# ISU-PAAL/DeepDFA

Hardware: NVIDIA H100
Metric: CFG graphs/sec (train step) (higher is better)
Workload: dtype f32 (GRU GEMMs: bf16x3 split operands, f32 accumulate)

## Files before the change

### deepdfa_b200/csrc/gru_tc_bwd.cu

```cuda
#include <cuda_fp16.h>

#include <atomic>

#include "tc_common.cuh"

namespace ddfa {
namespace tc2b {
using namespace tcc;

constexpr int kThreads = 320, kEpiWarps = 8;

constexpr int kGbWarps = 8;
struct GbRow {
  float4 d, hv, rr, zz, nn, gh;
  float deg;
  int tb, te;
};
__device__ __forceinline__ float4 bf16x4_to_f4(const uint2 &p) {
  return make_float4(__uint_as_float(p.x << 16), __uint_as_float(p.x & 0xffff0000u), __uint_as_float(p.y << 16), __uint_as_float(p.y & 0xffff0000u));
}
__device__ __forceinline__ void gb_load(GbRow &x, const float *__restrict__ dh_out, const float *__restrict__ h,
                                        const uint8_t *__restrict__ h_img_src, const float *__restrict__ gates,
                                        const uint4 *__restrict__ gates_packed, const int32_t *__restrict__ indptr,
                                        const int32_t *__restrict__ indptr_t, size_t plane, int64_t node, int col, bool ok,
                                        uint64_t pol_saved, uint64_t pol_dh) {
  x.tb = x.te = 0;
  if (ok) {
    if (indptr_t) { x.tb = __ldcg(indptr_t + node); x.te = __ldcg(indptr_t + node + 1); }
    const size_t off = (size_t)node * kD + col;
    x.d = ldg_cg_f4_hint(dh_out + off, pol_dh);
    uint2 hh = make_uint2(0u, 0u), hl = hh;
    uint4 g0 = make_uint4(0u, 0u, 0u, 0u), g1 = g0;
    if (h) x.hv = ldg_cg_f4_hint(h + off, pol_saved);
    else {
      hh = __ldcg(reinterpret_cast<const uint2 *>(h_img_src + image_offset(node, col, 0)));
      hl = __ldcg(reinterpret_cast<const uint2 *>(h_img_src + image_offset(node, col, 1)));
    }
    if (gates) {
      x.rr = ldg_cg_f4_hint(gates + off, pol_saved);
      x.zz = ldg_cg_f4_hint(gates + plane + off, pol_saved);
      x.nn = ldg_cg_f4_hint(gates + 2 * plane + off, pol_saved);
      x.gh = ldg_cg_f4_hint(gates + 3 * plane + off, pol_saved);
    } else {
      g0 = __ldcg(gates_packed + (off >> 1));
      g1 = __ldcg(gates_packed + (off >> 1) + 1);
    }
    x.deg = (float)(__ldcg(indptr + node + 1) - __ldcg(indptr + node));
    if (!h) {
      const float4 a = bf16x4_to_f4(hh), b = bf16x4_to_f4(hl);
      x.hv = make_float4(a.x + b.x, a.y + b.y, a.z + b.z, a.w + b.w);
    }
    if (!gates) {
      unpack_gates(make_uint2(g0.x, g0.y), x.rr.x, x.zz.x, x.nn.x, x.gh.x);
      unpack_gates(make_uint2(g0.z, g0.w), x.rr.y, x.zz.y, x.nn.y, x.gh.y);
      unpack_gates(make_uint2(g1.x, g1.y), x.rr.z, x.zz.z, x.nn.z, x.gh.z);
      unpack_gates(make_uint2(g1.z, g1.w), x.rr.w, x.zz.w, x.nn.w, x.gh.w);
    }
  }
}

__global__ void __launch_bounds__(32 * kGbWarps, 2) gate_bwd_image_kernel(const float *__restrict__ dh_out, const float *__restrict__ h,
                                                                          const uint8_t *__restrict__ h_img_src,
                                                                          const float *__restrict__ gates, const uint4 *__restrict__ gates_packed,
                                                                          const int32_t *__restrict__ indptr,
                                                                          const float *__restrict__ ds_in, const int32_t *__restrict__ indptr_t,
                                                                          const int32_t *__restrict__ indices_t,
                                                                          int32_t N, uint8_t *__restrict__ q_img, size_t img_stride,
                                                                          uint8_t *__restrict__ h_img, float *__restrict__ dhz,
                                                                          float *__restrict__ db_fold,
                                                                          float *__restrict__ db_ih, float *__restrict__ db_hh, float *__restrict__ bias_slots,
                                                                          int hints) {
  __shared__ float red[kGbWarps][7 * kD];
  const int lane = threadIdx.x & 31, warp = threadIdx.x >> 5;
  const int col = lane * 4;
  pdl_launch_dependents();
  pdl_wait();
  const uint64_t pol_saved = l2_policy((hints & 2) ? 1 : 0), pol_tmp = l2_policy((hints & 4) ? 2 : 0), pol_dh = l2_policy((hints & 8) ? 1 : 0);
  const size_t plane = (size_t)N * kD;
  float4 sum[7];
#pragma unroll
  for (int i = 0; i < 7; ++i) sum[i] = make_float4(0.f, 0.f, 0.f, 0.f);
  const int64_t Npad = ((int64_t)N + kTileM - 1) / kTileM * kTileM;
  const int64_t stride = (int64_t)gridDim.x * kGbWarps;

  auto finish = [&](const GbRow &x, int64_t node, bool ok) {
    float4 qr = make_float4(0.f, 0.f, 0.f, 0.f), qz = qr, qn = qr, qnr = qr, hv = qr;
    if (ok) {
      hv = x.hv;
      st_f4_hint(dhz + (size_t)node * kD + col, make_float4(x.d.x * x.zz.x, x.d.y * x.zz.y, x.d.z * x.zz.z, x.d.w * x.zz.w), pol_tmp);
#define BWDQ(f)                                                      \
  {                                                                  \
    const float dz_ = x.d.f * (x.hv.f - x.nn.f);                     \
    const float dn_ = x.d.f * (1.f - x.zz.f);                        \
    qn.f = dn_ * (1.f - x.nn.f * x.nn.f);                            \
    qz.f = dz_ * x.zz.f * (1.f - x.zz.f);                            \
    qr.f = qn.f * x.gh.f * x.rr.f * (1.f - x.rr.f);                  \
    qnr.f = qn.f * x.rr.f;                                           \
  }
      BWDQ(x) BWDQ(y) BWDQ(z) BWDQ(w)
#undef BWDQ
      f4_add(sum[0], qr); f4_add(sum[1], qz); f4_add(sum[2], qn); f4_add(sum[3], qnr);
      f4_fma(sum[4], x.deg, qr); f4_fma(sum[5], x.deg, qz); f4_fma(sum[6], x.deg, qn);
    }
    const size_t o_hi = image_offset(node, col, 0), o_lo = image_offset(node, col, 1);
    uint2 ph, pl;
    split4(qr, ph, pl);  *reinterpret_cast<uint2 *>(q_img + 0 * img_stride + o_hi) = ph; *reinterpret_cast<uint2 *>(q_img + 0 * img_stride + o_lo) = pl;
    split4(qz, ph, pl);  *reinterpret_cast<uint2 *>(q_img + 1 * img_stride + o_hi) = ph; *reinterpret_cast<uint2 *>(q_img + 1 * img_stride + o_lo) = pl;
    split4(qn, ph, pl);  *reinterpret_cast<uint2 *>(q_img + 2 * img_stride + o_hi) = ph; *reinterpret_cast<uint2 *>(q_img + 2 * img_stride + o_lo) = pl;
    split4(qnr, ph, pl); *reinterpret_cast<uint2 *>(q_img + 3 * img_stride + o_hi) = ph; *reinterpret_cast<uint2 *>(q_img + 3 * img_stride + o_lo) = pl;
    if (h_img) {
      split4(hv, ph, pl); *reinterpret_cast<uint2 *>(h_img + o_hi) = ph; *reinterpret_cast<uint2 *>(h_img + o_lo) = pl;
    }
  };

  for (int64_t node = (int64_t)blockIdx.x * kGbWarps + warp; node < Npad; node += 2 * stride) {
    const int64_t node2 = node + stride;
    GbRow a, b;
    const bool ok_a = node < N, ok_b = node2 < N;
    gb_load(a, dh_out, h, h_img_src, gates, gates_packed, indptr, indptr_t, plane, node, col, ok_a, pol_saved, pol_dh);
    gb_load(b, dh_out, h, h_img_src, gates, gates_packed, indptr, indptr_t, plane, node2, col, ok_b, pol_saved, pol_dh);
    if (indptr_t) {
      int ia[4], ib[4];
#pragma unroll
      for (int k = 0; k < 4; ++k) {
        ia[k] = (a.tb + k < a.te) ? __ldcg(indices_t + a.tb + k) : -1;
        ib[k] = (b.tb + k < b.te) ? __ldcg(indices_t + b.tb + k) : -1;
      }
      float4 va[4], vb[4];
#pragma unroll
      for (int k = 0; k < 4; ++k) {
        va[k] = ia[k] >= 0 ? ldg_cg_f4(ds_in + (size_t)ia[k] * kD + col) : make_float4(0.f, 0.f, 0.f, 0.f);
        vb[k] = ib[k] >= 0 ? ldg_cg_f4(ds_in + (size_t)ib[k] * kD + col) : make_float4(0.f, 0.f, 0.f, 0.f);
      }
#pragma unroll
      for (int k = 0; k < 4; ++k) { f4_add(a.d, va[k]); f4_add(b.d, vb[k]); }
      for (int j = a.tb + 4; j < a.te; ++j) f4_add(a.d, ldg_cg_f4(ds_in + (size_t)__ldcg(indices_t + j) * kD + col));
      for (int j = b.tb + 4; j < b.te; ++j) f4_add(b.d, ldg_cg_f4(ds_in + (size_t)__ldcg(indices_t + j) * kD + col));
    }
    finish(a, node, ok_a);
    if (node2 < Npad) finish(b, node2, ok_b);
  }
#pragma unroll
  for (int i = 0; i < 7; ++i) *reinterpret_cast<float4 *>(&red[warp][i * kD + col]) = sum[i];
  __syncthreads();
  for (int i = threadIdx.x; i < 7 * kD; i += 32 * kGbWarps) {
    float v_ = 0.f;
#pragma unroll
    for (int w = 0; w < kGbWarps; ++w) v_ += red[w][i];
    if (bias_slots) { bias_slots[(size_t)blockIdx.x * 7 * kD + i] = v_; continue; }
    const int which = i >> 7, c_ = i & 127;
    if (which == 0) { atomicAdd(db_ih + c_, v_); atomicAdd(db_hh + c_, v_); }
    else if (which == 1) { atomicAdd(db_ih + kD + c_, v_); atomicAdd(db_hh + kD + c_, v_); }
    else if (which == 2) atomicAdd(db_ih + 2 * kD + c_, v_);
    else if (which == 3) atomicAdd(db_hh + 2 * kD + c_, v_);
    else atomicAdd(db_fold + (which - 4) * kD + c_, v_);
  }
}

constexpr int kD3Stages = 2;
constexpr int kD3StageBytes = kImageTileBytes;
constexpr int kD3WChunkBytes = 64 * 128;
constexpr int kD3WBytes = 12 * kD3WChunkBytes;
constexpr int kD3OffStage = kD3WBytes;
constexpr int kD3OffBar = kD3OffStage + kD3Stages * kD3StageBytes;
constexpr int kD3SmemAlloc = kD3OffBar + (2 * kD3Stages + 1) * 8 + 1024;
constexpr int kD3Threads = 32 * kEpiWarps + 32;
constexpr size_t kD3PackedBytes = (size_t)4 * kD3WBytes;
static_assert(kD3SmemAlloc <= 232448, "shared memory budget");

__global__ void dgrad3_pack_kernel(const float *__restrict__ w_fold, const float *__restrict__ w_hh, uint8_t *__restrict__ packed) {
  const int idx = blockIdx.x * blockDim.x + threadIdx.x;
  if (idx >= 4 * 3 * 64 * 16) return;
  const int u = idx % 16, n = (idx / 16) % 64, g = (idx / (16 * 64)) % 3, rh = idx / (16 * 64 * 3);
  const int role = rh >> 1, half = rh & 1, kb = u >> 3;
  const float *W = role == 0 ? w_fold : w_hh;
  float x[8];
#pragma unroll
  for (int i = 0; i < 8; ++i) x[i] = W[(size_t)(g * kD + u * 8 + i) * kD + half * 64 + n];
  uint4 ph, pl;
  split8(x, ph, pl);
  uint8_t *base = packed + (size_t)rh * kD3WBytes + sw128_offset(n, (u & 7) * 8);
  *reinterpret_cast<uint4 *>(base + ((g * 2 + 0) * 2 + kb) * kD3WChunkBytes) = ph;
  *reinterpret_cast<uint4 *>(base + ((g * 2 + 1) * 2 + kb) * kD3WChunkBytes) = pl;
}

__global__ void __launch_bounds__(kD3Threads, 1) dgrad3_kernel(const uint8_t *__restrict__ q_img, size_t img_stride,
                                                               const float *__restrict__ dhz, const uint8_t *__restrict__ packed3,
                                                               int32_t N, float *__restrict__ ds, float *__restrict__ dh, int hints) {
  extern __shared__ uint8_t smem_raw[];
  uint8_t *smem = reinterpret_cast<uint8_t *>((reinterpret_cast<uintptr_t>(smem_raw) + 1023) & ~(uintptr_t)1023);
  const uint32_t sbase = smem_u32(smem);
  const uint32_t bar0 = sbase + kD3OffBar;
  auto full = [&](int i) { return bar0 + 8u * i; };
  auto empty = [&](int i) { return bar0 + 8u * (kD3Stages + i); };
  const uint32_t w_full = bar0 + 8u * (2 * kD3Stages);
  const int tron = (g_trace_on == 1);

  const int warp = threadIdx.x >> 5, lane = threadIdx.x & 31;
  const int rh = blockIdx.x & 3, role = rh >> 1, half = rh & 1;
  const int group = blockIdx.x >> 2, num_groups = gridDim.x >> 2;
  const int num_tiles = (N + kTileM - 1) / kTileM;
  const int my_tiles = (num_tiles > group) ? (num_tiles - 1 - group) / num_groups + 1 : 0;

  if (threadIdx.x == 0) {
    for (int i = 0; i < kD3Stages; ++i) { mbar_init(full(i), 1); mbar_init(empty(i), kEpiWarps); }
    mbar_init(w_full, 1);
    mbar_fence_init();
  }
  __syncthreads();
  if (threadIdx.x == 0) trace_stamp(tron, 0, 0);
  pdl_launch_dependents();

  if (warp == kEpiWarps) {
    if (my_tiles > 0 && elect_one()) {
      mbar_arrive_expect_tx(w_full, kD3WBytes);
      bulk_g2s(sbase, packed3 + (size_t)rh * kD3WBytes, kD3WBytes, w_full);
      pdl_wait();
      const uint64_t pol_q = l2_policy((hints & 64) ? 1 : 0);
      int cc = 0;
      for (int k = 0; k < my_tiles; ++k) {
        const int tile = num_tiles - 1 - (group + k * num_groups);
        for (int g = 0; g < 3; ++g, ++cc) {
          const int m = g < 2 ? g : (role == 0 ? 2 : 3);
          const int stage = cc % kD3Stages, use = cc / kD3Stages;
          if (use > 0) mbar_wait_bounded(empty(stage), (use - 1) & 1);
          mbar_arrive_expect_tx(full(stage), kD3StageBytes);
          bulk_g2s_hint(sbase + kD3OffStage + stage * kD3StageBytes, q_img + (size_t)m * img_stride + (size_t)tile * kImageTileBytes,
                        kD3StageBytes, full(stage), pol_q);
          if (g != 1) trace_stamp(tron, k, g == 0 ? 1 : 2);
        }
      }
    }
    return;
  }

  pdl_wait();
  if (my_tiles == 0) return;
  const int wg = warp >> 2;
  const int row0 = wg * 64 + (warp & 3) * 16 + (lane >> 2);
  const int col0 = half * 64 + 2 * (lane & 3);
  float *out = role == 0 ? ds : dh;
  const uint64_t pol_tmp = l2_policy((hints & 4) ? 2 : 0);
  const uint64_t pol_dhz = l2_policy((hints & 8) ? 1 : 0);
  mbar_wait_bounded(w_full, 0);
  const bool tr = (warp == 0 && lane == 0);
  int cc = 0, pending = -1;
  for (int k = 0; k < my_tiles; ++k) {
    const int tile = num_tiles - 1 - (group + k * num_groups);
    float acc[32];
    if (tr) { trace_stamp(tron, k, 7); trace_stamp(tron, k, 3); }
    for (int g = 0; g < 3; ++g, ++cc) {
      const int stage = cc % kD3Stages, use = cc / kD3Stages;
      mbar_wait_bounded(full(stage), use & 1);
      if (tr && g != 1) trace_stamp(tron, k, g == 0 ? 4 : 5);
      wgmma_fence();
      const uint32_t a0 = sbase + kD3OffStage + stage * kD3StageBytes + wg * 8192;
      const uint32_t w0 = sbase + g * 4 * kD3WChunkBytes;
#pragma unroll
      for (int kb = 0; kb < 2; ++kb) {
#pragma unroll
        for (int k4 = 0; k4 < 4; ++k4) {
          const uint64_t a_hi = gmma_desc(a0 + kb * kChunkBytes + k4 * 32), a_lo = gmma_desc(a0 + (2 + kb) * kChunkBytes + k4 * 32);
          const uint64_t b_hi = gmma_desc(w0 + kb * kD3WChunkBytes + k4 * 32), b_lo = gmma_desc(w0 + (2 + kb) * kD3WChunkBytes + k4 * 32);
          wgmma_n64<0, 0>(acc, a_hi, b_hi, (g == 0 && kb == 0 && k4 == 0) ? 0u : 1u);
          wgmma_n64<0, 0>(acc, a_hi, b_lo, 1u);
          wgmma_n64<0, 0>(acc, a_lo, b_hi, 1u);
        }
      }
      wgmma_commit();
      wgmma_wait<1>();
      __syncwarp();
      if (pending >= 0 && lane == 0) mbar_arrive(empty(pending));
      pending = stage;
    }
    float2 dv[2][8];
#pragma unroll
    for (int hh = 0; hh < 2; ++hh) {
      const int64_t node = (int64_t)tile * kTileM + row0 + 8 * hh;
#pragma unroll
      for (int j = 0; j < 8; ++j) {
        dv[hh][j] = make_float2(0.f, 0.f);
        if (role == 1 && node < N) {
          const float *p = dhz + node * kD + col0 + 8 * j;
          dv[hh][j] = make_float2(ldg_cg_f32_hint(p, pol_dhz), ldg_cg_f32_hint(p + 1, pol_dhz));
        }
      }
    }
    wgmma_wait<0>();
    wgmma_fence_regs(acc);
    if (tr) { trace_stamp(tron, k, 6); trace_stamp(tron, k, 8); }
    __syncwarp();
    if (lane == 0) mbar_arrive(empty(pending));
    pending = -1;
    if (tr) trace_stamp(tron, k, 9);
#pragma unroll
    for (int hh = 0; hh < 2; ++hh) {
      const int64_t node = (int64_t)tile * kTileM + row0 + 8 * hh;
      if (node < N) {
#pragma unroll
        for (int j = 0; j < 8; ++j)
          st_f2_hint(out + node * kD + col0 + 8 * j, make_float2(acc[4 * j + 2 * hh] + dv[hh][j].x, acc[4 * j + 2 * hh + 1] + dv[hh][j].y), pol_tmp);
      }
    }
    if (tr) trace_stamp(tron, k, 10);
  }
}

constexpr int kGtRows = 32;
constexpr int kGtOffD = 0, kGtOffG = kGtRows * kD * 4, kGtOffH = kGtOffG + kGtRows * kD * 8;
static_assert(kGtOffH + kGtRows * kD * 4 == kD3StageBytes, "phase A's operands fill exactly one stage");
static_assert(4 * kGtRows == kTileM, "four CTAs per tile");
constexpr int kGtPre = 2;
constexpr int kGtRowsPerWarp = kGtRows / kEpiWarps;

__device__ __forceinline__ void fence_proxy_async_global() { asm volatile("fence.proxy.async.global;" ::: "memory"); }
__device__ __forceinline__ void cluster_arrive_release() { asm volatile("barrier.cluster.arrive.release;" ::: "memory"); }
__device__ __forceinline__ void cluster_wait_acquire() { asm volatile("barrier.cluster.wait.acquire;" ::: "memory"); }

template <bool HF32, bool CSRP>
__global__ void __launch_bounds__(kD3Threads, 1) bwd_step_fused_kernel(const float *__restrict__ dh_out, const float *__restrict__ h,
                                                                       const uint8_t *__restrict__ h_img_src, const uint2 *__restrict__ gates_packed,
                                                                       const int32_t *__restrict__ indptr, const float *__restrict__ ds_in,
                                                                       const int32_t *__restrict__ indptr_t, const int32_t *__restrict__ indices_t,
                                                                       int32_t N, uint8_t *__restrict__ q_img, size_t img_stride,
                                                                       const uint8_t *__restrict__ packed3, float *__restrict__ ds, float *__restrict__ dh,
                                                                       float *__restrict__ db_fold, float *__restrict__ db_ih, float *__restrict__ db_hh,
                                                                       float *__restrict__ bias_slots, int hints) {
  extern __shared__ uint8_t smem_raw[];
  uint8_t *smem = reinterpret_cast<uint8_t *>((reinterpret_cast<uintptr_t>(smem_raw) + 1023) & ~(uintptr_t)1023);
  const uint32_t sbase = smem_u32(smem);
  const uint32_t bar0 = sbase + kD3OffBar;
  auto full = [&](int i) { return bar0 + 8u * i; };
  auto empty = [&](int i) { return bar0 + 8u * (kD3Stages + i); };
  const uint32_t w_full = bar0 + 8u * (2 * kD3Stages);
  const int tron = (g_trace_on == 1);

  const int warp = threadIdx.x >> 5, lane = threadIdx.x & 31;
  const int rh = blockIdx.x & 3, role = rh >> 1, half = rh & 1;
  const int cluster = blockIdx.x >> 2, num_clusters = gridDim.x >> 2;
  const int num_tiles = (N + kTileM - 1) / kTileM;
  const int my_tiles = (num_tiles > cluster) ? (num_tiles - 1 - cluster) / num_clusters + 1 : 0;
  const int tile0 = num_tiles - 1 - cluster;
  auto tile_of = [&](int k) { return tile0 - k * num_clusters; };

  if (threadIdx.x == 0) {
    for (int i = 0; i < kD3Stages; ++i) { mbar_init(full(i), 1); mbar_init(empty(i), kEpiWarps); }
    mbar_init(w_full, 1);
    mbar_fence_init();
  }
  __syncthreads();
  if (threadIdx.x == 0) trace_stamp(tron, 0, 0);
  pdl_launch_dependents();

  if (warp == kEpiWarps) {
    const uint64_t pol_saved = l2_policy((hints & 2) ? 1 : 0), pol_dh = l2_policy((hints & 8) ? 1 : 0);
    const uint64_t pol_q = l2_policy((hints & 64) ? 1 : 0);
    if (my_tiles > 0 && elect_one()) {
      mbar_arrive_expect_tx(w_full, kD3WBytes);
      bulk_g2s(sbase, packed3 + (size_t)rh * kD3WBytes, kD3WBytes, w_full);
    }
    __syncwarp();
    pdl_wait();
    int cc = 0;
    for (int k = 0; k < my_tiles; ++k, cc += 4) {
      const int tile = tile_of(k);
      if (elect_one()) {
        const int stage = cc % kD3Stages, use = cc / kD3Stages;
        if (use > 0) mbar_wait_bounded(empty(stage), (use - 1) & 1);
        const int64_t r0 = (int64_t)tile * kTileM + kGtRows * rh;
        const int valid = (int)max((int64_t)0, min((int64_t)kGtRows, (int64_t)N - r0));
        const uint32_t dst = sbase + kD3OffStage + stage * kD3StageBytes;
        const uint32_t bytes = (uint32_t)valid * (kD * 4 + kD * 8) + (HF32 ? (uint32_t)valid * kD * 4 : (uint32_t)kGtRows * kD * 4);
        mbar_arrive_expect_tx(full(stage), bytes);
        if (valid > 0) {
          bulk_g2s_hint(dst + kGtOffD, dh_out + r0 * kD, (uint32_t)valid * kD * 4, full(stage), pol_dh);
          bulk_g2s_hint(dst + kGtOffG, gates_packed + r0 * kD, (uint32_t)valid * kD * 8, full(stage), pol_saved);
        }
        if (HF32) {
          if (valid > 0) bulk_g2s_hint(dst + kGtOffH, h + r0 * kD, (uint32_t)valid * kD * 4, full(stage), pol_saved);
        } else {
          const uint8_t *t0 = h_img_src + (size_t)tile * kImageTileBytes + (size_t)(kGtRows * rh) * 128;
#pragma unroll
          for (int ch = 0; ch < 4; ++ch) bulk_g2s_hint(dst + kGtOffH + ch * (kGtRows * 128), t0 + (size_t)ch * kChunkBytes, kGtRows * 128, full(stage), pol_saved);
        }
      }
      __syncwarp();
      cluster_arrive_release();
      cluster_wait_acquire();
      if (elect_one()) {
        fence_proxy_async_global();
        for (int g = 0; g < 3; ++g) {
          const int m = g < 2 ? g : (role == 0 ? 2 : 3);
          const int c = cc + 1 + g, stage = c % kD3Stages, use = c / kD3Stages;
          if (use > 0) mbar_wait_bounded(empty(stage), (use - 1) & 1);
          mbar_arrive_expect_tx(full(stage), kD3StageBytes);
          bulk_g2s_hint(sbase + kD3OffStage + stage * kD3StageBytes, q_img + (size_t)m * img_stride + (size_t)tile * kImageTileBytes,
                        kD3StageBytes, full(stage), pol_q);
          if (g != 1) trace_stamp(tron, k, g == 0 ? 1 : 2);
        }
      }
      __syncwarp();
    }
  } else {
    pdl_wait();
    const int col = lane * 4;
#define DDFA_POL_TMP l2_policy((hints & 4) ? 2 : 0)
#define DDFA_POL_DHZ l2_policy((hints & 8) ? 1 : 0)
    const int wg = warp >> 2;
    const int row0 = wg * 64 + (warp & 3) * 16 + (lane >> 2);
    const int col0 = half * 64 + 2 * (lane & 3);
    const bool tr = (warp == 0 && lane == 0);
    float4 sum[7];
#pragma unroll
    for (int i = 0; i < 7; ++i) sum[i] = make_float4(0.f, 0.f, 0.f, 0.f);
    static_assert(kGtPre == 2 && kGtRowsPerWarp == 4, "lane slots below assume four rows per warp and two prefetched neighbours per row");
    auto node_of = [&](int tile, int r) { return (int64_t)tile * kTileM + kGtRows * rh + warp + kEpiWarps * r; };
    auto load_scalars = [&](int kk) -> int {
      int v = 0;
      if (kk < my_tiles && lane < 16) {
        const int64_t nd = node_of(tile_of(kk), (lane >> 1) & 3);
        const int32_t *base = lane < 8 ? indptr : indptr_t;
        if (nd < N && base) v = __ldcg(base + nd + (lane & 1));
      }
      return v;
    };
    auto load_ids = [&](int sc) -> int {
      const int r_ = (lane >> 1) & 3, q_ = lane & 1;
      const int tb_ = __shfl_sync(0xffffffffu, sc, 8 + 2 * r_), te_ = __shfl_sync(0xffffffffu, sc, 9 + 2 * r_);
      int v = -1;
      if (lane >= 16 && lane < 24 && tb_ + q_ < te_) v = __ldcg(indices_t + tb_ + q_);
      return v;
    };
    int sc_cur = 0, sc_next = 0, id_cur = -1;
    if constexpr (CSRP) {
      sc_cur = load_scalars(0); sc_next = load_scalars(1);
      id_cur = load_ids(sc_cur);
    }
    int cc = 0;
    for (int k = 0; k < my_tiles; ++k) {
      const int tile = tile_of(k);
      {
        const int stage = cc % kD3Stages, use = cc / kD3Stages;
        ++cc;
        const int64_t node0 = node_of(tile, 0);
        bool ok[kGtRowsPerWarp];
        int tb[kGtRowsPerWarp], te[kGtRowsPerWarp];
        float deg[kGtRowsPerWarp];
        int id[kGtRowsPerWarp][kGtPre];
        if constexpr (CSRP) {
          const int sc_next2 = load_scalars(k + 2);
          const int id_next = load_ids(sc_next);
#pragma unroll
          for (int r = 0; r < kGtRowsPerWarp; ++r) {
            ok[r] = node0 + kEpiWarps * r < N;
            deg[r] = (float)(__shfl_sync(0xffffffffu, sc_cur, 2 * r + 1) - __shfl_sync(0xffffffffu, sc_cur, 2 * r));
            tb[r] = __shfl_sync(0xffffffffu, sc_cur, 8 + 2 * r); te[r] = __shfl_sync(0xffffffffu, sc_cur, 9 + 2 * r);
#pragma unroll
            for (int q = 0; q < kGtPre; ++q) id[r][q] = __shfl_sync(0xffffffffu, id_cur, 16 + 2 * r + q);
          }
          sc_cur = sc_next; sc_next = sc_next2; id_cur = id_next;
        } else {
#pragma unroll
          for (int r = 0; r < kGtRowsPerWarp; ++r) {
            const int64_t nd = node0 + kEpiWarps * r;
            ok[r] = nd < N;
            tb[r] = te[r] = 0;
            deg[r] = 0.f;
            if (ok[r]) {
              deg[r] = (float)(__ldcg(indptr + nd + 1) - __ldcg(indptr + nd));
              if (indptr_t) { tb[r] = __ldcg(indptr_t + nd); te[r] = __ldcg(indptr_t + nd + 1); }
            }
          }
#pragma unroll
          for (int r = 0; r < kGtRowsPerWarp; ++r)
#pragma unroll
            for (int q = 0; q < kGtPre; ++q) id[r][q] = (tb[r] + q < te[r]) ? __ldcg(indices_t + tb[r] + q) : -1;
        }
        float4 gv[kGtRowsPerWarp][kGtPre];
#pragma unroll
        for (int r = 0; r < kGtRowsPerWarp; ++r)
#pragma unroll
          for (int q = 0; q < kGtPre; ++q) gv[r][q] = id[r][q] >= 0 ? ldg_cg_f4(ds_in + (size_t)id[r][q] * kD + col) : make_float4(0.f, 0.f, 0.f, 0.f);
        mbar_wait_bounded(full(stage), use & 1);
        const uint8_t *st = smem + kD3OffStage + stage * kD3StageBytes;
#pragma unroll
        for (int r = 0; r < kGtRowsPerWarp; ++r) {
          const int row = warp + kEpiWarps * r;
          float4 d = make_float4(0.f, 0.f, 0.f, 0.f), hv = d, rr = d, zz = d, nn = d, gh = d;
          if (ok[r]) {
            d = *reinterpret_cast<const float4 *>(st + kGtOffD + row * (kD * 4) + col * 4);
            const uint4 g0 = *reinterpret_cast<const uint4 *>(st + kGtOffG + row * (kD * 8) + col * 8);
            const uint4 g1 = *reinterpret_cast<const uint4 *>(st + kGtOffG + row * (kD * 8) + col * 8 + 16);
            unpack_gates(make_uint2(g0.x, g0.y), rr.x, zz.x, nn.x, gh.x);
            unpack_gates(make_uint2(g0.z, g0.w), rr.y, zz.y, nn.y, gh.y);
            unpack_gates(make_uint2(g1.x, g1.y), rr.z, zz.z, nn.z, gh.z);
            unpack_gates(make_uint2(g1.z, g1.w), rr.w, zz.w, nn.w, gh.w);
            if (HF32) {
              hv = *reinterpret_cast<const float4 *>(st + kGtOffH + row * (kD * 4) + col * 4);
            } else {
              const uint32_t off = (uint32_t)((col >> 6) * (kGtRows * 128) + row * 128 + (((((col & 63) >> 3) ^ (row & 7)) & 7) << 4) + (col & 7) * 2);
              const uint2 hh = *reinterpret_cast<const uint2 *>(st + kGtOffH + off);
              const uint2 hl = *reinterpret_cast<const uint2 *>(st + kGtOffH + 2 * (kGtRows * 128) + off);
              const float4 a = bf16x4_to_f4(hh), b = bf16x4_to_f4(hl);
              hv = make_float4(a.x + b.x, a.y + b.y, a.z + b.z, a.w + b.w);
            }
#pragma unroll
            for (int q = 0; q < kGtPre; ++q) f4_add(d, gv[r][q]);
            for (int j = tb[r] + kGtPre; j < te[r]; ++j) f4_add(d, ldg_cg_f4(ds_in + (size_t)__ldcg(indices_t + j) * kD + col));
          }
          float4 qr = make_float4(0.f, 0.f, 0.f, 0.f), qz = qr, qn = qr, qnr = qr;
          const int64_t node = node0 + kEpiWarps * r;
          if (ok[r]) {
            st_f4_hint(dh + (size_t)node * kD + col, make_float4(d.x * zz.x, d.y * zz.y, d.z * zz.z, d.w * zz.w), DDFA_POL_TMP);
#define BWDQ2(f)                                         \
  {                                                      \
    const float dz_ = d.f * (hv.f - nn.f);               \
    const float dn_ = d.f * (1.f - zz.f);                \
    qn.f = dn_ * (1.f - nn.f * nn.f);                    \
    qz.f = dz_ * zz.f * (1.f - zz.f);                    \
    qr.f = qn.f * gh.f * rr.f * (1.f - rr.f);            \
    qnr.f = qn.f * rr.f;                                 \
  }
            BWDQ2(x) BWDQ2(y) BWDQ2(z) BWDQ2(w)
#undef BWDQ2
            f4_add(sum[0], qr); f4_add(sum[1], qz); f4_add(sum[2], qn); f4_add(sum[3], qnr);
            f4_fma(sum[4], deg[r], qr); f4_fma(sum[5], deg[r], qz); f4_fma(sum[6], deg[r], qn);
          }
          const size_t o_hi = image_offset(node, col, 0), o_lo = image_offset(node, col, 1);
          uint2 ph, pl;
          split4(qr, ph, pl);  *reinterpret_cast<uint2 *>(q_img + 0 * img_stride + o_hi) = ph; *reinterpret_cast<uint2 *>(q_img + 0 * img_stride + o_lo) = pl;
          split4(qz, ph, pl);  *reinterpret_cast<uint2 *>(q_img + 1 * img_stride + o_hi) = ph; *reinterpret_cast<uint2 *>(q_img + 1 * img_stride + o_lo) = pl;
          split4(qn, ph, pl);  *reinterpret_cast<uint2 *>(q_img + 2 * img_stride + o_hi) = ph; *reinterpret_cast<uint2 *>(q_img + 2 * img_stride + o_lo) = pl;
          split4(qnr, ph, pl); *reinterpret_cast<uint2 *>(q_img + 3 * img_stride + o_hi) = ph; *reinterpret_cast<uint2 *>(q_img + 3 * img_stride + o_lo) = pl;
        }
        __syncwarp();
        if (lane == 0) mbar_arrive(empty(stage));
      }
      fence_proxy_async_global();
      cluster_arrive_release();
      cluster_wait_acquire();
      if (tr) trace_stamp(tron, k, 11);
      if (k == 0) mbar_wait_bounded(w_full, 0);
      float acc[32];
      int pending = -1;
      if (tr) { trace_stamp(tron, k, 7); trace_stamp(tron, k, 3); }
      for (int g = 0; g < 3; ++g, ++cc) {
        const int stage = cc % kD3Stages, use = cc / kD3Stages;
        mbar_wait_bounded(full(stage), use & 1);
        if (tr && g != 1) trace_stamp(tron, k, g == 0 ? 4 : 5);
        wgmma_fence();
        const uint32_t a0 = sbase + kD3OffStage + stage * kD3StageBytes + wg * 8192;
        const uint32_t w0 = sbase + g * 4 * kD3WChunkBytes;
#pragma unroll
        for (int kb = 0; kb < 2; ++kb) {
#pragma unroll
          for (int k4 = 0; k4 < 4; ++k4) {
            const uint64_t a_hi = gmma_desc(a0 + kb * kChunkBytes + k4 * 32), a_lo = gmma_desc(a0 + (2 + kb) * kChunkBytes + k4 * 32);
            const uint64_t b_hi = gmma_desc(w0 + kb * kD3WChunkBytes + k4 * 32), b_lo = gmma_desc(w0 + (2 + kb) * kD3WChunkBytes + k4 * 32);
            wgmma_n64<0, 0>(acc, a_hi, b_hi, (g == 0 && kb == 0 && k4 == 0) ? 0u : 1u);
            wgmma_n64<0, 0>(acc, a_hi, b_lo, 1u);
            wgmma_n64<0, 0>(acc, a_lo, b_hi, 1u);
          }
        }
        wgmma_commit();
        wgmma_wait<1>();
        __syncwarp();
        if (pending >= 0 && lane == 0) mbar_arrive(empty(pending));
        pending = stage;
      }
      float2 dv[8];
      auto fetch_dv = [&](int hh) {
        const uint64_t pol_dhz = DDFA_POL_DHZ;
        const int64_t node = (int64_t)tile * kTileM + row0 + 8 * hh;
#pragma unroll
        for (int j = 0; j < 8; ++j) {
          dv[j] = make_float2(0.f, 0.f);
          if (role == 1 && node < N) {
            const float *p = dh + node * kD + col0 + 8 * j;
            dv[j] = make_float2(ldg_cg_f32_hint(p, pol_dhz), ldg_cg_f32_hint(p + 1, pol_dhz));
          }
        }
      };
      fetch_dv(0);
      wgmma_wait<0>();
      wgmma_fence_regs(acc);
      if (tr) { trace_stamp(tron, k, 6); trace_stamp(tron, k, 8); }
      __syncwarp();
      if (lane == 0) mbar_arrive(empty(pending));
      if (tr) trace_stamp(tron, k, 9);
#pragma unroll
      for (int hh = 0; hh < 2; ++hh) {
        if (hh == 1) fetch_dv(1);
        const int64_t node = (int64_t)tile * kTileM + row0 + 8 * hh;
        if (node < N) {
          const uint64_t pol_tmp = DDFA_POL_TMP;
          float *out = role == 0 ? ds : dh;
#pragma unroll
          for (int j = 0; j < 8; ++j)
            st_f2_hint(out + node * kD + col0 + 8 * j, make_float2(acc[4 * j + 2 * hh] + dv[j].x, acc[4 * j + 2 * hh + 1] + dv[j].y), pol_tmp);
        }
      }
      if (tr) trace_stamp(tron, k, 10);
    }
#undef DDFA_POL_TMP
#undef DDFA_POL_DHZ
    asm volatile("bar.sync 1, %0;" ::"n"(32 * kEpiWarps) : "memory");
    float *red = reinterpret_cast<float *>(smem + kD3OffStage);
#pragma unroll
    for (int i = 0; i < 7; ++i) *reinterpret_cast<float4 *>(&red[(warp * 7 + i) * kD + col]) = sum[i];
  }
  __syncthreads();
  const float *red = reinterpret_cast<const float *>(smem + kD3OffStage);
  for (int i = threadIdx.x; i < 7 * kD; i += kD3Threads) {
    float v_ = 0.f;
#pragma unroll
    for (int w = 0; w < kEpiWarps; ++w) v_ += red[(w * 7) * kD + i];
    if (bias_slots) { bias_slots[(size_t)blockIdx.x * 7 * kD + i] = v_; continue; }
    const int which = i >> 7, c_ = i & 127;
    if (which == 0) { atomicAdd(db_ih + c_, v_); atomicAdd(db_hh + c_, v_); }
    else if (which == 1) { atomicAdd(db_ih + kD + c_, v_); atomicAdd(db_hh + kD + c_, v_); }
    else if (which == 2) atomicAdd(db_ih + 2 * kD + c_, v_);
    else if (which == 3) atomicAdd(db_hh + 2 * kD + c_, v_);
    else atomicAdd(db_fold + (which - 4) * kD + c_, v_);
  }
}

constexpr int kWgSlotBytes = kImageTileBytes;
constexpr int kWgSlots = 3;
constexpr int kWgOffBar = kWgSlots * kWgSlotBytes;
constexpr int kWgSmemAlloc = kWgOffBar + 2 * kWgSlots * 8 + 1024;
constexpr int kWgThreads = 32 * kEpiWarps + 32;
constexpr size_t kWgPartialFloats = (size_t)3 * kD * kD;
constexpr int kWgMaxSteps = 16;
struct WgBatch {
  const uint8_t *s_img[kWgMaxSteps];
  const uint8_t *h_img[kWgMaxSteps];
  int32_t steps;
};
__global__ void __launch_bounds__(kWgThreads, 1) wgrad_kernel(const uint8_t *__restrict__ q_img, size_t img_stride, size_t step_stride,
                                                              const __grid_constant__ WgBatch batch,
                                                              int32_t N, float *__restrict__ partial, int first, int hints) {
  extern __shared__ uint8_t smem_raw[];
  uint8_t *smem = reinterpret_cast<uint8_t *>((reinterpret_cast<uintptr_t>(smem_raw) + 1023) & ~(uintptr_t)1023);
  const uint32_t sbase = smem_u32(smem);
  const uint32_t bar0 = sbase + kWgOffBar;
  auto full = [&](int i) { return bar0 + 8u * i; };
  auto empty = [&](int i) { return bar0 + 8u * (kWgSlots + i); };

  const int warp = threadIdx.x >> 5, lane = threadIdx.x & 31;
  const int role = blockIdx.y / 3, g = blockIdx.y % 3;
  const int qm = g < 2 ? g : (role == 0 ? 2 : 3);
  const int num_tiles = (N + kTileM - 1) / kTileM;
  const int all_tiles = num_tiles * batch.steps;
  const int my_tiles = (all_tiles > (int)blockIdx.x) ? (all_tiles - 1 - (int)blockIdx.x) / (int)gridDim.x + 1 : 0;

  if (threadIdx.x == 0) {
    for (int i = 0; i < kWgSlots; ++i) { mbar_init(full(i), 1); mbar_init(empty(i), kEpiWarps); }
    mbar_fence_init();
  }
  __syncthreads();
  const int tron = (g_trace_on == 2) && blockIdx.y == 0;
  if (threadIdx.x == 0) trace_stamp(tron, 0, 0);

  if (warp == kEpiWarps) {
    if (elect_one()) {
      const uint64_t pol_wg = l2_policy((hints & 32) ? 1 : 0);
      for (int i = 0; i < my_tiles; ++i) {
        const int idx = (int)blockIdx.x + i * (int)gridDim.x;
        const int t = idx / num_tiles, tile = idx - t * num_tiles;
        for (int w = 0; w < 2; ++w) {
          const int cc = 2 * i + w, slot = cc % kWgSlots, use = cc / kWgSlots;
          if (use > 0) mbar_wait_bounded(empty(slot), (use - 1) & 1);
          const uint8_t *src = w == 0 ? (role == 0 ? batch.s_img[t] : batch.h_img[t]) : q_img + (size_t)t * step_stride + (size_t)qm * img_stride;
          mbar_arrive_expect_tx(full(slot), kWgSlotBytes);
          bulk_g2s_hint(sbase + slot * kWgSlotBytes, src + (size_t)tile * kImageTileBytes, kWgSlotBytes, full(slot), pol_wg);
          trace_stamp(tron, i, 1 + w);
        }
      }
    }
    return;
  }

  const int wg = warp >> 2;
  float acc[64], sum[64];
#pragma unroll
  for (int i = 0; i < 64; ++i) acc[i] = sum[i] = 0.f;
  for (int i = 0; i < my_tiles; ++i) {
    const int cb = 2 * i, ca = 2 * i + 1;
    mbar_wait_bounded(full(cb % kWgSlots), (cb / kWgSlots) & 1);
    if (warp == 0 && lane == 0) trace_stamp(tron, i, 3);
    mbar_wait_bounded(full(ca % kWgSlots), (ca / kWgSlots) & 1);
    if (warp == 0 && lane == 0) { trace_stamp(tron, i, 4); trace_stamp(tron, i, 5); }
    const uint32_t b0 = sbase + (cb % kWgSlots) * kWgSlotBytes;
    const uint32_t a0 = sbase + (ca % kWgSlots) * kWgSlotBytes + wg * kChunkBytes;
    constexpr uint32_t vs = 2 * kChunkBytes;
    wgmma_fence();
#pragma unroll
    for (int k16 = 0; k16 < kTileM / 16; ++k16) {
      const uint32_t koff = (uint32_t)k16 * 2048u;
      const uint64_t a_hi = gmma_desc(a0 + koff, kChunkBytes), a_lo = gmma_desc(a0 + vs + koff, kChunkBytes);
      const uint64_t b_hi = gmma_desc(b0 + koff, kChunkBytes), b_lo = gmma_desc(b0 + vs + koff, kChunkBytes);
      wgmma_n128<1, 1>(acc, a_hi, b_hi, k16 == 0 ? 0u : 1u);
      wgmma_n128<1, 1>(acc, a_lo, b_hi, 1u);
      wgmma_n128<1, 1>(acc, a_hi, b_lo, 1u);
    }
    wgmma_commit();
    if (warp == 0 && lane == 0) trace_stamp(tron, i, 6);
    wgmma_wait<0>();
    wgmma_fence_regs(acc);
    __syncwarp();
    if (lane == 0) { mbar_arrive(empty(cb % kWgSlots)); mbar_arrive(empty(ca % kWgSlots)); }
#pragma unroll
    for (int j = 0; j < 64; ++j) sum[j] += acc[j];
  }
  if (warp == 0 && lane == 0) trace_stamp(tron, 0, 8);
  float *dst = partial + ((size_t)role * gridDim.x + blockIdx.x) * kWgPartialFloats;
  const int row0 = g * kD + wg * 64 + (warp & 3) * 16 + (lane >> 2);
#pragma unroll
  for (int hh = 0; hh < 2; ++hh) {
    float *rowp = dst + (size_t)(row0 + 8 * hh) * kD + 2 * (lane & 3);
#pragma unroll
    for (int j = 0; j < 16; ++j) {
      float2 v = make_float2(sum[4 * j + 2 * hh], sum[4 * j + 2 * hh + 1]);
      if (!first) {
        const float2 o = *reinterpret_cast<const float2 *>(rowp + 8 * j);
        v.x += o.x;
        v.y += o.y;
      }
      *reinterpret_cast<float2 *>(rowp + 8 * j) = v;
    }
  }
  if (warp == 0 && lane == 0) trace_stamp(tron, 0, 10);
}

__global__ void __launch_bounds__(256) wgrad_reduce_kernel(const float *__restrict__ partial, int ctas, float *__restrict__ dw_fold,
                                                           float *__restrict__ dw_hh) {
  const int i = blockIdx.x * blockDim.x + threadIdx.x;
  const int role = blockIdx.y;
  if (i >= (int)(kWgPartialFloats / 4)) return;
  const float4 *src = reinterpret_cast<const float4 *>(partial + (size_t)role * ctas * kWgPartialFloats) + i;
  float4 s = make_float4(0.f, 0.f, 0.f, 0.f);
  for (int c = 0; c < ctas; ++c) f4_add(s, src[(size_t)c * (kWgPartialFloats / 4)]);
  float4 *dst = reinterpret_cast<float4 *>(role == 0 ? dw_fold : dw_hh) + i;
  float4 d = *dst;
  f4_add(d, s);
  *dst = d;
}

constexpr int kBiasSlots = 2 * kNumSMs;
__global__ void __launch_bounds__(128) bias_slots_reduce_kernel(const float *__restrict__ slots, int ctas, float *__restrict__ db_fold,
                                                                float *__restrict__ db_ih, float *__restrict__ db_hh) {
  const int i = blockIdx.x * 128 + threadIdx.x;
  const int which = i >> 7, c_ = i & 127;
  float v_ = 0.f;
  for (int c = 0; c < ctas; ++c) v_ += slots[(size_t)c * 7 * kD + i];
  if (which == 0) { db_ih[c_] += v_; db_hh[c_] += v_; }
  else if (which == 1) { db_ih[kD + c_] += v_; db_hh[kD + c_] += v_; }
  else if (which == 2) db_ih[2 * kD + c_] += v_;
  else if (which == 3) db_hh[2 * kD + c_] += v_;
  else db_fold[(which - 4) * kD + c_] += v_;
}

}

constexpr int kWgCtas = kNumSMs / 6;
static size_t wg_partial_bytes() { return (size_t)2 * kWgCtas * tc2b::kWgPartialFloats * sizeof(float); }
int gru_tc2b_trace_enable(int on) {
  DDFA_CUDA(cudaMemcpyToSymbol(tcc::g_trace_on, &on, sizeof(int)));
  return DDFA_OK;
}
int gru_tc2b_trace_read(void *host, size_t bytes) {
  if (bytes > tcc::kTraceWords * sizeof(long long)) bytes = tcc::kTraceWords * sizeof(long long);
  DDFA_CUDA(cudaMemcpyFromSymbol(host, tcc::g_trace, bytes));
  return DDFA_OK;
}
static constexpr size_t kPackedTotal = tc2b::kD3PackedBytes;
static constexpr size_t kBiasSlotBytes = (size_t)tc2b::kBiasSlots * 7 * tcc::kD * sizeof(float);
static size_t bwd_fixed_bytes(int32_t N) { return kPackedTotal + 3 * tcc::image_bytes(N) + wg_partial_bytes() + kBiasSlotBytes; }
void *gru_tc2_bwd_s_image_scratch(void *workspace, int32_t N) { return static_cast<uint8_t *>(workspace) + kPackedTotal + 2 * tcc::image_bytes(N); }
size_t gru_tc2_bwd_workspace_bytes(int32_t N, int32_t slots) {
  return bwd_fixed_bytes(N) + (size_t)(slots < 1 ? 1 : slots) * 4 * tcc::image_bytes(N);
}


int gru_tc2_prepare_bwd(const float *w_fold, const float *w_hh, void *workspace, size_t workspace_bytes, cudaStream_t stream) {
  if (workspace == nullptr || workspace_bytes < kPackedTotal) {
    set_error("tcgen05 engine (bwd): workspace too small");
    return DDFA_ERR_WORKSPACE;
  }
  const int total = 4 * 3 * 64 * 16;
  tc2b::dgrad3_pack_kernel<<<(total + 127) / 128, 128, 0, stream>>>(w_fold, w_hh, static_cast<uint8_t *>(workspace));
  DDFA_CHECK_LAUNCH("tc2b::dgrad3_pack_kernel");
  chain_break();
  return DDFA_OK;
}

int gru_tc2_bwd_finish(int32_t N, float *dw_fold, float *dw_hh, void *workspace, size_t workspace_bytes, cudaStream_t stream) {
  if (workspace == nullptr || workspace_bytes < gru_tc2_bwd_workspace_bytes(N, 1)) {
    set_error("tcgen05 engine (bwd finish): workspace too small");
    return DDFA_ERR_WORKSPACE;
  }
  float *partial = reinterpret_cast<float *>(static_cast<uint8_t *>(workspace) + kPackedTotal + 3 * tcc::image_bytes(N));
  const int n4 = (int)(tc2b::kWgPartialFloats / 4);
  tc2b::wgrad_reduce_kernel<<<dim3((n4 + 255) / 256, 2), 256, 0, stream>>>(partial, kWgCtas, dw_fold, dw_hh);
  DDFA_CHECK_LAUNCH("tc2b::wgrad_reduce_kernel");
  return DDFA_OK;
}

template <bool HF32, bool CSRP>
static int bwd_fused_max_clusters(int *out) {
  static std::atomic<int> cached{0};
  int v = cached.load(std::memory_order_relaxed);
  if (v == 0) {
    DDFA_CUDA(cudaFuncSetAttribute(tc2b::bwd_step_fused_kernel<HF32, CSRP>, cudaFuncAttributeMaxDynamicSharedMemorySize, tc2b::kD3SmemAlloc));
    cudaLaunchConfig_t cfg = {};
    cfg.gridDim = dim3(kNumSMs / 4 * 4);
    cfg.blockDim = dim3(tc2b::kD3Threads);
    cfg.dynamicSmemBytes = tc2b::kD3SmemAlloc;
    cudaLaunchAttribute attr;
    attr.id = cudaLaunchAttributeClusterDimension;
    attr.val.clusterDim.x = 4;
    attr.val.clusterDim.y = 1;
    attr.val.clusterDim.z = 1;
    cfg.attrs = &attr;
    cfg.numAttrs = 1;
    DDFA_CUDA(cudaOccupancyMaxActiveClusters(&v, tc2b::bwd_step_fused_kernel<HF32, CSRP>, &cfg));
    if (v < 1) {
      set_error("tcgen05 engine (bwd): bwd_step_fused_kernel fits no 4-CTA cluster on this device");
      return DDFA_ERR_CUDA;
    }
    cached.store(v, std::memory_order_relaxed);
  }
  *out = v;
  return DDFA_OK;
}
int gru_tc2b_fused_max_clusters(int *out) { return bwd_fused_max_clusters<false, true>(out); }

template <bool HF32, bool CSRP>
static int launch_bwd_fused(int tiles, cudaStream_t stream, const float *dh_out, const float *h, const void *h_img_in, const void *gates_packed,
                            const int32_t *indptr, const float *ds_in, const int32_t *indptr_t, const int32_t *indices_t, int32_t N,
                            uint8_t *q_img, size_t img, const uint8_t *packed, float *ds, float *dh, float *db_fold, float *db_ih, float *db_hh,
                            float *bias_slots, int *ctas) {
  int clusters = 0;
  const int rc = bwd_fused_max_clusters<HF32, CSRP>(&clusters);
  if (rc != DDFA_OK) return rc;
  if (clusters > tiles) clusters = tiles;
  *ctas = clusters * 4;
  DDFA_REQUIRE(bias_slots == nullptr || *ctas <= tc2b::kBiasSlots, "tcgen05 engine (bwd): %d CTAs exceed the %d bias-gradient slots",
               *ctas, tc2b::kBiasSlots);
  DDFA_CUDA(cudaFuncSetAttribute(tc2b::bwd_step_fused_kernel<HF32, CSRP>, cudaFuncAttributeMaxDynamicSharedMemorySize, tc2b::kD3SmemAlloc));
  DDFA_CUDA(launch_chain_cluster(4, 4, tc2b::bwd_step_fused_kernel<HF32, CSRP>, dim3(clusters * 4), dim3(tc2b::kD3Threads), tc2b::kD3SmemAlloc,
                                 stream, dh_out, h, static_cast<const uint8_t *>(h_img_in), static_cast<const uint2 *>(gates_packed), indptr,
                                 ds_in, ds_in ? indptr_t : nullptr, indices_t, N, q_img, img, packed, ds, dh, db_fold, db_ih, db_hh, bias_slots,
                                 l2_hints()));
  DDFA_CHECK_LAUNCH("tc2b::bwd_step_fused_kernel");
  return DDFA_OK;
}

int gru_tc2_step_bwd(const float *dh_out, const float *ds_in, const int32_t *indptr_t, const int32_t *indices_t, const float *h,
                     const void *h_img_in, const void *s_img, const float *gates, const void *gates_packed, const int32_t *indptr, int32_t N, float *ds, float *dh, float *dw_fold, float *db_fold, float *db_ih,
                     float *dw_hh, float *db_hh, void *workspace, size_t workspace_bytes, int wgrad_mode, cudaStream_t stream) {
  if (h == nullptr && h_img_in == nullptr) {
    set_error("tcgen05 engine (bwd): neither the fp32 h nor its activation image given");
    return DDFA_ERR_INVALID_ARG;
  }
  const int q_slot = wgrad_mode >= 16 ? wgrad_mode - 16 : 0;
  if (workspace == nullptr || workspace_bytes < gru_tc2_bwd_workspace_bytes(N, q_slot + 1)) {
    set_error("tcgen05 engine (bwd): workspace too small (%zu < %zu)", workspace_bytes, gru_tc2_bwd_workspace_bytes(N, q_slot + 1));
    return DDFA_ERR_WORKSPACE;
  }
  uint8_t *packed = static_cast<uint8_t *>(workspace);
  const size_t img = tcc::image_bytes(N);
  uint8_t *h_img_ws = packed + kPackedTotal;
  float *partial = reinterpret_cast<float *>(h_img_ws + 3 * img);
  float *bias_slots = deterministic() ? reinterpret_cast<float *>(h_img_ws + 3 * img + wg_partial_bytes()) : nullptr;
  int ctas = 0;
  uint8_t *q_img = packed + bwd_fixed_bytes(N) + (size_t)q_slot * 4 * img;
  const uint8_t *h_img = h_img_in ? static_cast<const uint8_t *>(h_img_in) : h_img_ws;
  const int tiles = (N + tcc::kTileM - 1) / tcc::kTileM;
  if (gates_packed && gate_bwd_tma()) {
    const bool csrp = gate_bwd_tma() >= 2;
    int rc = DDFA_OK;
    if (h) rc = csrp ? launch_bwd_fused<true, true>(tiles, stream, dh_out, h, h_img_in, gates_packed, indptr, ds_in, indptr_t, indices_t, N, q_img, img, packed, ds, dh, db_fold, db_ih, db_hh, bias_slots, &ctas)
                     : launch_bwd_fused<true, false>(tiles, stream, dh_out, h, h_img_in, gates_packed, indptr, ds_in, indptr_t, indices_t, N, q_img, img, packed, ds, dh, db_fold, db_ih, db_hh, bias_slots, &ctas);
    else   rc = csrp ? launch_bwd_fused<false, true>(tiles, stream, dh_out, h, h_img_in, gates_packed, indptr, ds_in, indptr_t, indices_t, N, q_img, img, packed, ds, dh, db_fold, db_ih, db_hh, bias_slots, &ctas)
                     : launch_bwd_fused<false, false>(tiles, stream, dh_out, h, h_img_in, gates_packed, indptr, ds_in, indptr_t, indices_t, N, q_img, img, packed, ds, dh, db_fold, db_ih, db_hh, bias_slots, &ctas);
    if (rc != DDFA_OK) return rc;
  } else {
    const int64_t rows = (int64_t)tiles * tcc::kTileM;
    const int64_t want = (rows + tc2b::kGbWarps - 1) / tc2b::kGbWarps;
    const unsigned gb_grid = (unsigned)(want < tc2b::kBiasSlots ? want : tc2b::kBiasSlots);
    ctas = (int)gb_grid;
    float *dhz = reinterpret_cast<float *>(h_img_ws + img);
    DDFA_CUDA(launch_chain(4, tc2b::gate_bwd_image_kernel, dim3(gb_grid), dim3(32 * tc2b::kGbWarps), 0, stream, dh_out, h,
                           static_cast<const uint8_t *>(h_img_in), gates, static_cast<const uint4 *>(gates_packed), indptr, ds_in,
                           ds_in ? indptr_t : nullptr, indices_t, N, q_img, img, h_img_in ? nullptr : h_img_ws, dhz, db_fold, db_ih, db_hh,
                           bias_slots, l2_hints()));
    DDFA_CHECK_LAUNCH("tc2b::gate_bwd_image_kernel");
    DDFA_CUDA(cudaFuncSetAttribute(tc2b::dgrad3_kernel, cudaFuncAttributeMaxDynamicSharedMemorySize, tc2b::kD3SmemAlloc));
    int groups = kNumSMs / 4;
    if (groups > tiles) groups = tiles;
    DDFA_CUDA(launch_chain(8, tc2b::dgrad3_kernel, dim3(groups * 4), dim3(tc2b::kD3Threads), tc2b::kD3SmemAlloc, stream, q_img, img, dhz,
                           static_cast<const uint8_t *>(packed), N, ds, dh, l2_hints()));
    DDFA_CHECK_LAUNCH("tc2b::dgrad3_kernel");
  }
  if (bias_slots) {
    tc2b::bias_slots_reduce_kernel<<<7, 128, 0, stream>>>(bias_slots, ctas, db_fold, db_ih, db_hh);
    DDFA_CHECK_LAUNCH("tc2b::bias_slots_reduce_kernel");
  }
  DDFA_CUDA(cudaFuncSetAttribute(tc2b::wgrad_kernel, cudaFuncAttributeMaxDynamicSharedMemorySize, tc2b::kWgSmemAlloc));
  if (wgrad_mode >= 16) return DDFA_OK;
  tc2b::WgBatch one = {};
  one.s_img[0] = static_cast<const uint8_t *>(s_img);
  one.h_img[0] = h_img;
  one.steps = 1;
  tc2b::wgrad_kernel<<<dim3(kWgCtas, 6), tc2b::kWgThreads, tc2b::kWgSmemAlloc, stream>>>(q_img, img, 0, one, N, partial, wgrad_mode == 2 ? 0 : 1, 0);
  DDFA_CHECK_LAUNCH("tc2b::wgrad_kernel");
  if (wgrad_mode == 0) return gru_tc2_bwd_finish(N, dw_fold, dw_hh, workspace, workspace_bytes, stream);
  return DDFA_OK;
}

int gru_tc2_bwd_wgrad_batched(const void *const *s_imgs, const void *const *h_imgs, int32_t steps, int32_t N, float *dw_fold,
                              float *dw_hh, void *workspace, size_t workspace_bytes, cudaStream_t stream) {
  if (steps < 1 || steps > tc2b::kWgMaxSteps) {
    set_error("tcgen05 engine (batched wgrad): 1 <= steps <= %d required (got %d)", tc2b::kWgMaxSteps, steps);
    return DDFA_ERR_INVALID_ARG;
  }
  if (workspace == nullptr || workspace_bytes < gru_tc2_bwd_workspace_bytes(N, steps)) {
    set_error("tcgen05 engine (batched wgrad): workspace too small (%zu < %zu)", workspace_bytes, gru_tc2_bwd_workspace_bytes(N, steps));
    return DDFA_ERR_WORKSPACE;
  }
  uint8_t *packed = static_cast<uint8_t *>(workspace);
  const size_t img = tcc::image_bytes(N);
  float *partial = reinterpret_cast<float *>(packed + kPackedTotal + 3 * img);
  const uint8_t *q_img = packed + bwd_fixed_bytes(N);
  tc2b::WgBatch b = {};
  for (int t = 0; t < steps; ++t) {
    if (!s_imgs[t] || !h_imgs[t]) {
      set_error("tcgen05 engine (batched wgrad): NULL image pointer for step %d", t);
      return DDFA_ERR_INVALID_ARG;
    }
    b.s_img[t] = static_cast<const uint8_t *>(s_imgs[t]);
    b.h_img[t] = static_cast<const uint8_t *>(h_imgs[t]);
  }
  b.steps = steps;
  DDFA_CUDA(cudaFuncSetAttribute(tc2b::wgrad_kernel, cudaFuncAttributeMaxDynamicSharedMemorySize, tc2b::kWgSmemAlloc));
  tc2b::wgrad_kernel<<<dim3(kWgCtas, 6), tc2b::kWgThreads, tc2b::kWgSmemAlloc, stream>>>(q_img, img, 4 * img, b, N, partial, 1, l2_hints());
  DDFA_CHECK_LAUNCH("tc2b::wgrad_kernel");
  return gru_tc2_bwd_finish(N, dw_fold, dw_hh, workspace, workspace_bytes, stream);
}

}
```

Baseline: 114,700.

## Stage GEMM epilogue through shared memory and emit bulk TMA stores/reduce-adds

```diff
diff --git a/deepdfa_b200/csrc/gru_tc_bwd.cu b/deepdfa_b200/csrc/gru_tc_bwd.cu
--- a/deepdfa_b200/csrc/gru_tc_bwd.cu
+++ b/deepdfa_b200/csrc/gru_tc_bwd.cu
@@ -314,8 +314,32 @@
 constexpr int kGtRowsPerWarp = kGtRows / kEpiWarps;
 
 __device__ __forceinline__ void fence_proxy_async_global() { asm volatile("fence.proxy.async.global;" ::: "memory"); }
+__device__ __forceinline__ void fence_proxy_async_shared() { asm volatile("fence.proxy.async.shared::cta;" ::: "memory"); }
 __device__ __forceinline__ void cluster_arrive_release() { asm volatile("barrier.cluster.arrive.release;" ::: "memory"); }
 __device__ __forceinline__ void cluster_wait_acquire() { asm volatile("barrier.cluster.wait.acquire;" ::: "memory"); }
+__device__ __forceinline__ void mbar_arrive_n(uint32_t bar, uint32_t n) {
+  asm volatile("mbarrier.arrive.shared::cta.b64 _, [%0], %1;" ::"r"(bar), "r"(n) : "memory");
+}
+__device__ __forceinline__ void bulk_s2g_hint(float *dst, uint32_t src, uint32_t bytes, uint64_t pol) {
+  asm volatile("cp.async.bulk.global.shared::cta.bulk_group.L2::cache_hint [%0], [%1], %2, %3;" ::"l"(dst), "r"(src), "r"(bytes), "l"(pol)
+               : "memory");
+}
+__device__ __forceinline__ void bulk_s2g_add_f32_hint(float *dst, uint32_t src, uint32_t bytes, uint64_t pol) {
+  asm volatile("cp.reduce.async.bulk.global.shared::cta.bulk_group.L2::cache_hint.add.f32 [%0], [%1], %2, %3;" ::"l"(dst), "r"(src),
+               "r"(bytes), "l"(pol)
+               : "memory");
+}
+__device__ __forceinline__ void bulk_commit() { asm volatile("cp.async.bulk.commit_group;" ::: "memory"); }
+__device__ __forceinline__ void bulk_wait_read_all() { asm volatile("cp.async.bulk.wait_group.read 0;" ::: "memory"); }
+__device__ __forceinline__ void bulk_wait_all() { asm volatile("cp.async.bulk.wait_group 0;" ::: "memory"); }
+
+constexpr int kD3OutStage = 3 % kD3Stages;
+static_assert(4 % kD3Stages == 0, "q2 lands in the same stage every tile");
+constexpr int kStRowBytes = 64 * 4 + 16;
+static_assert(16 * kStRowBytes <= kChunkBytes / 2, "16 staged rows fit in a warpgroup's half of a chunk");
+__device__ __forceinline__ uint32_t staged_row(uint32_t stage, int wg, int r) {
+  return stage + (uint32_t)((r >> 4) * kChunkBytes + wg * (kChunkBytes / 2) + (r & 15) * kStRowBytes);
+}
 
 template <bool HF32, bool CSRP>
 __global__ void __launch_bounds__(kD3Threads, 1) bwd_step_fused_kernel(const float *__restrict__ dh_out, const float *__restrict__ h,
@@ -405,10 +429,7 @@
     pdl_wait();
     const int col = lane * 4;
 #define DDFA_POL_TMP l2_policy((hints & 4) ? 2 : 0)
-#define DDFA_POL_DHZ l2_policy((hints & 8) ? 1 : 0)
     const int wg = warp >> 2;
-    const int row0 = wg * 64 + (warp & 3) * 16 + (lane >> 2);
-    const int col0 = half * 64 + 2 * (lane & 3);
     const bool tr = (warp == 0 && lane == 0);
     float4 sum[7];
 #pragma unroll
@@ -536,10 +557,16 @@
         __syncwarp();
         if (lane == 0) mbar_arrive(empty(stage));
       }
+      if (k > 0 && (warp & 3) == 0) {
+        bulk_wait_read_all();
+        __syncwarp();
+        if (lane == 0) mbar_arrive_n(empty(kD3OutStage), kEpiWarps / 2);
+      }
       fence_proxy_async_global();
       cluster_arrive_release();
       cluster_wait_acquire();
       if (tr) trace_stamp(tron, k, 11);
+      if ((warp & 3) == 0 && role == 1) fence_proxy_async_global();
       if (k == 0) mbar_wait_bounded(w_full, 0);
       float acc[32];
       int pending = -1;
@@ -568,42 +595,40 @@
         if (pending >= 0 && lane == 0) mbar_arrive(empty(pending));
         pending = stage;
       }
-      float2 dv[8];
-      auto fetch_dv = [&](int hh) {
-        const uint64_t pol_dhz = DDFA_POL_DHZ;
-        const int64_t node = (int64_t)tile * kTileM + row0 + 8 * hh;
-#pragma unroll
-        for (int j = 0; j < 8; ++j) {
-          dv[j] = make_float2(0.f, 0.f);
-          if (role == 1 && node < N) {
-            const float *p = dh + node * kD + col0 + 8 * j;
-            dv[j] = make_float2(ldg_cg_f32_hint(p, pol_dhz), ldg_cg_f32_hint(p + 1, pol_dhz));
-          }
-        }
-      };
-      fetch_dv(0);
       wgmma_wait<0>();
       wgmma_fence_regs(acc);
-      if (tr) { trace_stamp(tron, k, 6); trace_stamp(tron, k, 8); }
+      if (tr) { trace_stamp(tron, k, 6); trace_stamp(tron, k, 8); trace_stamp(tron, k, 9); }
+      const uint32_t st_base = sbase + kD3OffStage + kD3OutStage * kD3StageBytes;
+      if (wg == 0) asm volatile("bar.sync 2, 128;" ::: "memory");
+      else asm volatile("bar.sync 3, 128;" ::: "memory");
+      uint32_t tid;
+      asm volatile("mov.u32 %0, %%tid.x;" : "=r"(tid));
+#pragma unroll
+      for (int hh = 0; hh < 2; ++hh) {
+        const uint32_t rowp = staged_row(st_base, wg, (tid >> 5 & 3) * 16 + (tid >> 2 & 7) + 8 * hh) + 8 * (tid & 3);
+#pragma unroll
+        for (int j = 0; j < 8; ++j)
+          asm volatile("st.shared.v2.f32 [%0], {%1, %2};" ::"r"(rowp + 32 * j), "f"(acc[4 * j + 2 * hh]), "f"(acc[4 * j + 2 * hh + 1]) : "memory");
+      }
+      fence_proxy_async_shared();
+      if (wg == 0) asm volatile("bar.sync 2, 128;" ::: "memory");
+      else asm volatile("bar.sync 3, 128;" ::: "memory");
+      if ((warp & 3) == 0 && elect_one()) {
+        const uint64_t pol_tmp = DDFA_POL_TMP;
+        const int64_t node0 = (int64_t)tile * kTileM + wg * 64;
+        float *out = (role == 0 ? ds : dh) + node0 * kD + half * 64;
+        const int rows = (int)min((int64_t)64, (int64_t)N - node0);
+        for (int r = 0; r < rows; ++r) {
+          if (role == 0) bulk_s2g_hint(out + (int64_t)r * kD, staged_row(st_base, wg, r), 64 * 4, pol_tmp);
+          else bulk_s2g_add_f32_hint(out + (int64_t)r * kD, staged_row(st_base, wg, r), 64 * 4, pol_tmp);
+        }
+        bulk_commit();
+      }
       __syncwarp();
-      if (lane == 0) mbar_arrive(empty(pending));
-      if (tr) trace_stamp(tron, k, 9);
-#pragma unroll
-      for (int hh = 0; hh < 2; ++hh) {
-        if (hh == 1) fetch_dv(1);
-        const int64_t node = (int64_t)tile * kTileM + row0 + 8 * hh;
-        if (node < N) {
-          const uint64_t pol_tmp = DDFA_POL_TMP;
-          float *out = role == 0 ? ds : dh;
-#pragma unroll
-          for (int j = 0; j < 8; ++j)
-            st_f2_hint(out + node * kD + col0 + 8 * j, make_float2(acc[4 * j + 2 * hh] + dv[j].x, acc[4 * j + 2 * hh + 1] + dv[j].y), pol_tmp);
-        }
-      }
       if (tr) trace_stamp(tron, k, 10);
     }
 #undef DDFA_POL_TMP
-#undef DDFA_POL_DHZ
+    bulk_wait_all();
     asm volatile("bar.sync 1, %0;" ::"n"(32 * kEpiWarps) : "memory");
     float *red = reinterpret_cast<float *>(smem + kD3OffStage);
 #pragma unroll
```

After: 120,000, median of 6. +4.6%, better.
